# ai-forever/Kandinsky-2

Measured on NVIDIA H100. Metric: unet_denoising_steps_per_sec, higher is better.
Workload: dtype f16

## Files before the change

kandinsky-2_b200/csrc/k2_api.cu:

```cuda
#include <stdio.h>
#include <stdlib.h>
#include <string.h>

#include <algorithm>
#include <atomic>
#include <mutex>

#include "../../include/k2b200.h"
#include "k2_internal.h"

namespace k2 {

static thread_local std::string g_err;
static std::atomic<long long> g_launches{0};
static int g_force_bn = 0;
static int g_force_split = 0;
static int g_pdl = 0;


void set_error(const std::string& msg) { g_err = msg; }
int fail(const std::string& msg) {
  g_err = msg;
  return -1;
}
void count_launch(int n) { g_launches.fetch_add(n, std::memory_order_relaxed); }

bool pdl_enabled() { return g_pdl != 0; }
static int g_conv_epi_sets = 1;
static int g_gn_bps = 0;
int gn_apply_blocks_per_sm() { return g_gn_bps; }
static int g_attn_half = 1;
int attention_half_rows() { return g_attn_half; }

int num_sms() {
  static int n = 0;
  if (n == 0) {
    int dev = 0;
    cudaGetDevice(&dev);
    cudaDeviceGetAttribute(&n, cudaDevAttrMultiProcessorCount, dev);
    if (n <= 0) n = 132;
  }
  return n;
}

typedef CUresult (*EncodeTiledFn)(CUtensorMap*, CUtensorMapDataType, cuuint32_t, void*, const cuuint64_t*,
                                  const cuuint64_t*, const cuuint32_t*, const cuuint32_t*,
                                  CUtensorMapInterleave, CUtensorMapSwizzle, CUtensorMapL2promotion,
                                  CUtensorMapFloatOOBfill);

static EncodeTiledFn get_encode_fn() {
  static EncodeTiledFn fn = nullptr;
  static std::once_flag once;
  std::call_once(once, [] {
    void* p = nullptr;
    cudaDriverEntryPointQueryResult qres;
    cudaError_t e = cudaGetDriverEntryPoint("cuTensorMapEncodeTiled", &p, cudaEnableDefault, &qres);
    if (e == cudaSuccess && qres == cudaDriverEntryPointSuccess) fn = reinterpret_cast<EncodeTiledFn>(p);
  });
  return fn;
}

int encode_tmap_f16(CUtensorMap* out, const void* base, int rank, const uint64_t* dims,
                    const uint64_t* strides_bytes, const uint32_t* box) {
  EncodeTiledFn fn = get_encode_fn();
  if (!fn) return fail("cuTensorMapEncodeTiled unavailable (no CUDA driver)");
  cuuint64_t gdim[5];
  cuuint64_t gstr[4];
  cuuint32_t bx[5];
  cuuint32_t es[5];
  for (int i = 0; i < rank; ++i) {
    gdim[i] = dims[i];
    bx[i] = box[i];
    es[i] = 1;
  }
  for (int i = 0; i + 1 < rank; ++i) gstr[i] = strides_bytes[i];
  CUresult r = fn(out, CU_TENSOR_MAP_DATA_TYPE_FLOAT16, static_cast<cuuint32_t>(rank), const_cast<void*>(base),
                  gdim, gstr, bx, es, CU_TENSOR_MAP_INTERLEAVE_NONE, CU_TENSOR_MAP_SWIZZLE_128B,
                  CU_TENSOR_MAP_L2_PROMOTION_L2_256B, CU_TENSOR_MAP_FLOAT_OOB_FILL_NONE);
  if (r != CUDA_SUCCESS) {
    char buf[256];
    snprintf(buf, sizeof buf,
             "cuTensorMapEncodeTiled failed (%d): rank %d dims %llu %llu %llu %llu box %u %u %u %u base %p",
             static_cast<int>(r), rank, (unsigned long long)dims[0], (unsigned long long)(rank > 1 ? dims[1] : 0),
             (unsigned long long)(rank > 2 ? dims[2] : 0), (unsigned long long)(rank > 3 ? dims[3] : 0), box[0],
             rank > 1 ? box[1] : 0, rank > 2 ? box[2] : 0, rank > 3 ? box[3] : 0, base);
    return fail(buf);
  }
  return 0;
}

static void choose_tile(int NB, int H, int W, int& TN, int& TH, int& TW, bool single_image_only = false) {
  long long best_tiles[2] = {-1, -1};
  int bn[2] = {1, 1}, bw[2] = {1, 1}, bh[2] = {1, 1};
  const int wmax = W < 128 ? W : 128;
  for (int tw = 1; tw <= wmax; ++tw) {
    const long long tiles_w = (W + tw - 1) / tw;
    for (int tn = 1; tn <= NB && tn * tw <= 128; ++tn) {
      int thmax = 128 / (tw * tn);
      if (thmax > H) thmax = H;
      if (thmax < 1) continue;
      const long long tiles_h = (H + thmax - 1) / thmax;
      const int th = static_cast<int>((H + tiles_h - 1) / tiles_h);
      const long long tiles = tiles_h * tiles_w * ((NB + tn - 1) / tn);
      for (int k = (tn == 1 ? 0 : 1); k < 2; ++k) {
        bool better = best_tiles[k] < 0 || tiles < best_tiles[k];
        if (!better && tiles == best_tiles[k]) {
          if (tn != bn[k]) {
            better = tn < bn[k];
          } else {
            const int d_new = tw > th ? tw - th : th - tw;
            const int d_old = bw[k] > bh[k] ? bw[k] - bh[k] : bh[k] - bw[k];
            better = (d_new < d_old) || (d_new == d_old && tw > bw[k]);
          }
        }
        if (better) {
          best_tiles[k] = tiles;
          bn[k] = tn;
          bw[k] = tw;
          bh[k] = th;
        }
      }
    }
  }
  const int k = (!single_image_only && best_tiles[1] * 100 <= best_tiles[0] * 85) ? 1 : 0;
  TN = bn[k];
  TW = bw[k];
  TH = bh[k];
}


struct ConvPlan {
  int TN, TH, TW, tiles_w, tiles_h, tiles_n, m_tiles;
  int m_tiles_phase;
  int BN, splits;
  int fuse_stats, row_groups;
  int es;
};

static void plan_conv(int NB, int H, int W, bool any9, int kchunks, int Cout, int out_mode, bool has_workspace,
                      long long workspace_bytes, bool want_gn, ConvPlan& pl, const int* cfg = nullptr, bool up2 = false,
                      bool w_batched = false) {
  const int g_force_bn = (cfg && cfg[0]) ? cfg[0] : k2::g_force_bn;
  const int g_force_split = (cfg && cfg[2]) ? cfg[2] : k2::g_force_split;
  pl.es = (cfg && cfg[3]) ? cfg[3] : k2::g_conv_epi_sets;
  choose_tile(NB, H, W, pl.TN, pl.TH, pl.TW, w_batched);
  pl.tiles_w = (W + pl.TW - 1) / pl.TW;
  pl.tiles_h = (H + pl.TH - 1) / pl.TH;
  pl.tiles_n = (NB + pl.TN - 1) / pl.TN;
  pl.m_tiles = pl.tiles_w * pl.tiles_h * pl.tiles_n;
  pl.m_tiles_phase = pl.m_tiles;

  int BN = g_force_bn;
  int splits = 1;
  const long long M_total = static_cast<long long>(NB) * H * W;
  const bool can_split = !up2 && !w_batched && has_workspace && out_mode == 0 && Cout % 8 == 0;
  auto split_ok = [&](int sp) {
    if (sp == 1) return true;
    const int kps = (kchunks + sp - 1) / sp;
    return can_split && kps >= 8 && (sp - 1) * kps < kchunks &&
           static_cast<long long>(sp) * M_total * Cout * 4 <= workspace_bytes;
  };
  auto model = [&](int bn, int sp) {
    const long long nt = (Cout + bn - 1) / bn;
    const long long units = static_cast<long long>(pl.m_tiles) * nt * sp * (up2 ? 4 : 1);
    const long long slots = num_sms();
    const long long waves = (units + slots - 1) / slots;
    const long long kps = (kchunks + sp - 1) / sp;
    long long cost = waves * (kps * (4LL * bn + 60) + 2000);
    if (sp > 1) cost += 4000 + (static_cast<long long>(sp) + 1) * M_total * Cout * 4 / 1800;
    return cost;
  };
  if (BN == 0) {
    if (Cout <= 16) BN = 16;
    else if (Cout <= 64) BN = 64;
    else if (Cout <= 128) BN = 128;
    else BN = 0;
  }
  {
    const int cand[3] = {256, 192, 128};
    long long best = -1;
    int best_bn = BN ? BN : 256, best_sp = 1;
    for (int ci = 0; ci < 3; ++ci) {
      const int bn = BN ? BN : cand[ci];
      if (BN && ci > 0) break;
      for (int sp = 1; sp <= 8; ++sp) {
        if (g_force_split > 0 && sp != g_force_split) continue;
        if (!split_ok(sp)) continue;
        const long long c = model(bn, sp);
        if (best < 0 || c < best) {
          best = c;
          best_bn = bn;
          best_sp = sp;
        }
      }
    }
    BN = best_bn;
    splits = best_sp;
  }
  pl.BN = BN;
  pl.splits = splits;

  pl.fuse_stats = 0;
  pl.row_groups = 0;
  if (want_gn && out_mode == 0 && Cout % 8 == 0) {
    if (splits == 1 && BN >= 64 && Cout % 64 == 0 && (pl.TN == 1 || pl.TH * pl.TW == 16)) {
      pl.fuse_stats = 1;
      pl.row_groups = ((pl.TN == 1) ? pl.m_tiles : NB * pl.tiles_h * pl.tiles_w) * (up2 ? 4 : 1);
    } else if (splits > 1 && (static_cast<long long>(H) * W) % 16 == 0) {
      pl.fuse_stats = 2;
      pl.row_groups = static_cast<int>(M_total / 16);
    }
  }
}

static void plan_to_info(const ConvPlan& pl, int* info) {
  if (!info) return;
  info[0] = pl.BN; info[1] = 0;
  info[2] = pl.splits; info[3] = pl.m_tiles; info[4] = pl.TN;
  info[5] = pl.fuse_stats; info[6] = pl.row_groups;
}

}

using namespace k2;

extern "C" {

const char* k2_last_error(void) { return g_err.c_str(); }
int k2_version(void) { return 100; }
long long k2_launch_count(void) { return g_launches.load(); }
void k2_reset_launch_count(void) { g_launches.store(0); }
int k2_set_tuning(int key, int value) {
  if (key == 0) {
    g_force_bn = value;
    return 0;
  }
  if (key == 1) {
    g_force_split = value;
    return 0;
  }
  if (key == 2) {
    if (value == 2) return fail("k2_set_tuning: no CTA-pair conv kernel on sm_90");
    return 0;
  }
  if (key == 4) {
    g_pdl = value;
    return 0;
  }
  if (key == 10) {
    g_conv_epi_sets = (value == 2) ? 2 : 1;
    return 0;
  }
  if (key == 11) {
    g_gn_bps = value;
    return 0;
  }
  if (key == 9) {
    g_attn_half = value ? 1 : 0;
    return 0;
  }

  return fail("k2_set_tuning: unknown key");
}

int k2_conv_gemm(const K2ConvSrc* srcs, int nsrc, int NB, int H, int W, const void* w_packed, int w_rows,
                 int Ktot, int ldw, int Cout, const float* bias, const void* residual, int ldr, void* out, int ldo,
                 int out_mode, void* workspace, long long workspace_bytes, float* gn_partial, int* info,
                 k2_stream_t stream) {
  return k2_conv_gemm_cfg(srcs, nsrc, NB, H, W, w_packed, w_rows, Ktot, ldw, Cout, bias, residual, ldr, out, ldo, out_mode,
                          workspace, workspace_bytes, gn_partial, info, nullptr, 0, stream);
}

int k2_conv_gemm_cfg(const K2ConvSrc* srcs, int nsrc, int NB, int H, int W, const void* w_packed, int w_rows,
                     int Ktot, int ldw, int Cout, const float* bias, const void* residual, int ldr, void* out, int ldo,
                     int out_mode, void* workspace, long long workspace_bytes, float* gn_partial, int* info,
                     const int* cfg, long long w_batch_stride, k2_stream_t stream) {
  K2_REQUIRE(w_batch_stride >= 0 && w_batch_stride % 8 == 0, "conv_gemm_cfg: w_batch_stride must be a multiple of 8 elements");
  const bool w_batched = w_batch_stride > 0;
  if (cfg) {
    K2_REQUIRE(cfg[0] == 0 || cfg[0] == 16 || cfg[0] == 64 || cfg[0] == 128 || cfg[0] == 192 || cfg[0] == 256,
               "conv_gemm_cfg: N tile must be 0, 16, 64, 128, 192 or 256");
    K2_REQUIRE(cfg[1] >= 0 && cfg[1] <= 2 && cfg[2] >= 0 && cfg[2] <= 8 && cfg[3] >= 0 && cfg[3] <= 2,
               "conv_gemm_cfg: pair mode in 0..2, splits in 0..8, epilogue sets in 0..2");
    K2_REQUIRE(cfg[1] != 2, "conv_gemm_cfg: no CTA-pair conv kernel on sm_90");
  }
  K2_REQUIRE(nsrc >= 1 && nsrc <= 3, "conv_gemm: 1..3 sources");
  K2_REQUIRE((reinterpret_cast<uintptr_t>(gn_partial) & 7) == 0, "conv_gemm: gn_partial must be 8-byte aligned");
  K2_REQUIRE(NB > 0 && H > 0 && W > 0 && Cout > 0, "conv_gemm: bad geometry");
  K2_REQUIRE(w_rows >= Cout, "conv_gemm: w_rows < Cout");
  K2_REQUIRE(Ktot % 64 == 0, "conv_gemm: Ktot must be a multiple of 64");
  if (ldw == 0) ldw = Ktot;
  K2_REQUIRE(ldw >= Ktot && ldw % 8 == 0 && (reinterpret_cast<uintptr_t>(w_packed) & 15) == 0,
             "conv_gemm: weight row stride / alignment");
  ConvGemmParams p;
  memset(&p, 0, sizeof p);
  p.NB = NB;
  p.H = H;
  p.W = W;
  bool any9 = false;
  int kchunks = 0;
  const bool up2 = srcs[0].taps == 4;
  if (up2) {
    K2_REQUIRE(nsrc == 1 && out_mode == 0 && residual == nullptr && H % 2 == 0 && W % 2 == 0,
               "conv_gemm: a taps == 4 source (3x3 conv over its nearest-2x upsampling) must be the only source, with fp16 "
               "output, no residual and even output H, W");
    H /= 2;
    W /= 2;
    p.H = H;
    p.W = W;
  }
  for (int s = 0; s < nsrc; ++s) {
    const K2ConvSrc& src = srcs[s];
    K2_REQUIRE(src.taps == 9 || src.taps == 1 || (s == 0 && src.taps == 4), "conv_gemm: taps must be 9 or 1 (or 4: up2)");
    K2_REQUIRE(src.C > 0 && src.C % 8 == 0 && src.ld % 8 == 0 && src.ld >= src.C, "conv_gemm: bad source C/ld");
    K2_REQUIRE((reinterpret_cast<uintptr_t>(src.ptr) & 15) == 0, "conv_gemm: source not 16B aligned");
    any9 = any9 || src.taps == 9;
    p.seg_taps[s] = src.taps;
    p.seg_kchunks[s] = (src.C + 63) / 64;
    kchunks += src.taps * p.seg_kchunks[s];
  }
  K2_REQUIRE(kchunks * 64 * (up2 ? 4 : 1) == Ktot,
             "conv_gemm: Ktot does not match the sources (taps * ceil(C/64)*64 summed; x4 phases for a taps == 4 source)");
  p.num_k_chunks = kchunks;

  ConvPlan pl;
  plan_conv(NB, H, W, any9 || up2, kchunks, Cout, out_mode, workspace != nullptr, workspace_bytes, gn_partial != nullptr, pl,
            cfg, up2, w_batched);
  K2_REQUIRE(!w_batched || (!up2 && pl.TN == 1), "conv_gemm_cfg: batched weights need single-image tiles");
  p.w_batched = w_batched ? 1 : 0;
  plan_to_info(pl, info);
  p.TN = pl.TN;
  p.TH = pl.TH;
  p.TW = pl.TW;
  p.tiles_w = pl.tiles_w;
  p.tiles_h = pl.tiles_h;
  p.tiles_n = pl.tiles_n;
  p.m_tiles = up2 ? 4 * pl.m_tiles_phase : pl.m_tiles;
  p.m_tiles_phase = pl.m_tiles_phase;
  p.up2 = up2 ? 1 : 0;
  p.a_box_bytes = static_cast<uint32_t>(p.TN * p.TH * p.TW * 128);
  for (int s = 0; s < nsrc; ++s) {
    const K2ConvSrc& src = srcs[s];
    uint64_t dims[4] = {static_cast<uint64_t>(src.C), static_cast<uint64_t>(W), static_cast<uint64_t>(H),
                        static_cast<uint64_t>(NB)};
    uint64_t str[3] = {static_cast<uint64_t>(src.ld) * 2, static_cast<uint64_t>(src.ld) * 2 * W,
                       static_cast<uint64_t>(src.ld) * 2 * W * H};
    uint32_t box[4] = {64, static_cast<uint32_t>(p.TW), static_cast<uint32_t>(p.TH), static_cast<uint32_t>(p.TN)};
    if (encode_tmap_f16(&p.tmA[s], src.ptr, 4, dims, str, box)) return -1;
  }
  const int BN = pl.BN, splits = pl.splits, fuse_stats = pl.fuse_stats;
  p.splits = splits;
  p.k_per_split = (kchunks + splits - 1) / splits;
  p.M_total = static_cast<long long>(NB) * H * W * (up2 ? 4 : 1);
  p.ws = reinterpret_cast<float*>(workspace);
  p.n_tiles = (Cout + BN - 1) / BN;
  p.Cout = Cout;
  {
    uint64_t dims[3] = {static_cast<uint64_t>(Ktot), static_cast<uint64_t>(w_rows), static_cast<uint64_t>(w_batched ? NB : 1)};
    uint64_t str[2] = {static_cast<uint64_t>(ldw) * 2,
                       (w_batched ? static_cast<uint64_t>(w_batch_stride) : static_cast<uint64_t>(ldw) * w_rows) * 2};
    uint32_t box[3] = {64, static_cast<uint32_t>(BN), 1};
    if (encode_tmap_f16(&p.tmB, w_packed, 3, dims, str, box)) return -1;
  }
  p.bias = bias;
  p.residual = reinterpret_cast<const __half*>(residual);
  p.ldr = ldr;
  p.out = out;
  p.ldo = ldo;
  p.out_mode = (splits > 1) ? 2 : out_mode;
  p.gn_part = (fuse_stats == 1) ? reinterpret_cast<float2*>(gn_partial) : nullptr;
  p.gn_mode = (fuse_stats == 1) ? (p.TN == 1 ? 1 : 2) : 0;
  if (out_mode == 0) {
    K2_REQUIRE(ldo % 8 == 0 && (reinterpret_cast<uintptr_t>(out) & 15) == 0, "conv_gemm: out alignment");
    if (residual)
      K2_REQUIRE(ldr % 8 == 0 && (reinterpret_cast<uintptr_t>(residual) & 15) == 0, "conv_gemm: residual alignment");
  }
  int rc = launch_conv_gemm(p, BN, pl.es, static_cast<cudaStream_t>(stream));
  if (rc == 0) g_launches.fetch_add(1, std::memory_order_relaxed);
  if (rc == 0 && splits > 1) {
    rc = launch_splitk_finalize(p.ws, splits, p.M_total, Cout, bias, p.residual, ldr, reinterpret_cast<__half*>(out), ldo,
                                fuse_stats == 2 ? reinterpret_cast<float2*>(gn_partial) : nullptr,
                                static_cast<cudaStream_t>(stream));
    if (rc == 0) g_launches.fetch_add(1, std::memory_order_relaxed);
  }
  return rc;
}

int k2_conv_plan(int NB, int H, int W, int taps, int Ktot, int Cout, int out_mode, long long workspace_bytes,
                 int want_gn_partial, int* info) {
  K2_REQUIRE(NB > 0 && H > 0 && W > 0 && Cout > 0 && info, "conv_plan: bad arguments");
  K2_REQUIRE(Ktot > 0 && Ktot % 64 == 0, "conv_plan: Ktot must be a positive multiple of 64");
  ConvPlan pl;
  plan_conv(NB, H, W, taps == 9, Ktot / 64, Cout, out_mode, workspace_bytes > 0, workspace_bytes, want_gn_partial != 0, pl);
  plan_to_info(pl, info);
  return 0;
}

}
```

kandinsky-2_b200/csrc/k2_attention.cu:

```cuda
#include <string.h>

#include <algorithm>

#include "../../include/k2b200.h"
#include "k2_common.cuh"
#include "k2_internal.h"

namespace k2 {

namespace {

__device__ __forceinline__ float ex2(float x) {
  float y;
  asm("ex2.approx.ftz.f32 %0, %1;" : "=f"(y) : "f"(x));
  return y;
}
__device__ __forceinline__ uint32_t pack_h2(float lo, float hi) {
  __half2 h = __floats2half2_rn(lo, hi);
  return *reinterpret_cast<uint32_t*>(&h);
}

template <int D, int DV, int NW, int BKV>
struct FlashCfg {
  static constexpr int BQ = 16 * NW;
  static constexpr int QP = D + 8;
  static constexpr int VP = DV + 8;
  static constexpr int Q_BYTES = BQ * QP * 2;
  static constexpr int K_BYTES = BKV * QP * 2;
  static constexpr int V_BYTES = BKV * VP * 2;
  static constexpr int SMEM_BYTES = Q_BYTES + 2 * (K_BYTES + V_BYTES);
};

template <int D, int DV, int NW, int BKV>
__global__ void __launch_bounds__(NW * 32, 1) flash_attention_kernel(const FlashParams p) {
  using C = FlashCfg<D, DV, NW, BKV>;
  constexpr int NSPLIT = D / DV;
  extern __shared__ __align__(16) uint8_t smem[];
  __half* sQ = reinterpret_cast<__half*>(smem);
  __half* sK = reinterpret_cast<__half*>(smem + C::Q_BYTES);
  __half* sV = reinterpret_cast<__half*>(smem + C::Q_BYTES + 2 * C::K_BYTES);

  const int tid = threadIdx.x;
  const int warp = tid >> 5;
  const int lane = tid & 31;
  const int q0 = blockIdx.x * C::BQ;
  const int head = blockIdx.y / NSPLIT;
  const int dsplit = blockIdx.y - head * NSPLIT;
  const int b = blockIdx.z;
  const int Tkv = p.Tc + p.T;
  const int nblk = (Tkv + BKV - 1) / BKV;

  pdl_wait();
  pdl_launch();

  {
    constexpr int CPR = D / 8;
    for (int i = tid; i < C::BQ * CPR; i += NW * 32) {
      const int r = i / CPR, c = i - r * CPR;
      const int q = q0 + r;
      const __half* src = p.qkv + (static_cast<long long>(b) * p.T + (q < p.T ? q : 0)) * p.ldq + head * p.hs + p.q_off + c * 8;
      cp_async_16(smem_u32(sQ + r * C::QP + c * 8), src, q < p.T ? 16 : 0);
    }
  }
  auto load_kv = [&](int jb, int st) {
    constexpr int KC = D / 8, VC = DV / 8;
    for (int i = tid; i < BKV * (KC + VC); i += NW * 32) {
      const int r = i / (KC + VC), c = i - r * (KC + VC);
      const int key = jb * BKV + r;
      const bool ok = key < Tkv;
      const bool from_enc = key < p.Tc;
      const __half* row = from_enc ? p.enc + (static_cast<long long>(b) * p.Tc + key) * p.lde + head * p.ehs
                                   : p.qkv + (static_cast<long long>(b) * p.T + (ok ? key - p.Tc : 0)) * p.ldq + head * p.hs;
      if (c < KC) {
        const __half* src = row + (from_enc ? p.ek_off : p.k_off) + c * 8;
        cp_async_16(smem_u32(sK + (st * BKV + r) * C::QP + c * 8), ok ? src : p.qkv, ok ? 16 : 0);
      } else {
        const __half* src = row + (from_enc ? p.ev_off : p.v_off) + dsplit * DV + (c - KC) * 8;
        cp_async_16(smem_u32(sV + (st * BKV + r) * C::VP + (c - KC) * 8), ok ? src : p.qkv, ok ? 16 : 0);
      }
    }
  };
  load_kv(0, 0);
  cp_async_commit();

  const float c = p.scale_log2e;
  float m_r[2] = {-INFINITY, -INFINITY}, l_r[2] = {0.f, 0.f};
  float o[DV / 8][4];
#pragma unroll
  for (int n = 0; n < DV / 8; ++n) o[n][0] = o[n][1] = o[n][2] = o[n][3] = 0.f;

  const uint32_t q_lane = smem_u32(sQ + (warp * 16 + (lane & 15)) * C::QP + (lane >> 4) * 8);
  for (int jb = 0; jb < nblk; ++jb) {
    const int st = jb & 1;
    if (jb + 1 < nblk) {
      load_kv(jb + 1, st ^ 1);
      cp_async_commit();
      cp_async_wait<1>();
    } else {
      cp_async_wait<0>();
    }
    __syncthreads();

    float s[BKV / 8][4];
#pragma unroll
    for (int n = 0; n < BKV / 8; ++n) s[n][0] = s[n][1] = s[n][2] = s[n][3] = 0.f;
    const uint32_t k_lane = smem_u32(sK + (st * BKV + ((lane >> 4) << 3) + (lane & 7)) * C::QP + ((lane >> 3) & 1) * 8);
#pragma unroll 4
    for (int kk = 0; kk < D / 16; ++kk) {
      uint32_t a[4];
      ldmatrix_x4(a, q_lane + kk * 32);
#pragma unroll
      for (int n = 0; n < BKV / 8; n += 2) {
        uint32_t bk[4];
        ldmatrix_x4(bk, k_lane + n * 8 * C::QP * 2 + kk * 32);
        mma_16816(s[n], a, bk[0], bk[1]);
        mma_16816(s[n + 1], a, bk[2], bk[3]);
      }
    }

    const int kbase = jb * BKV + 2 * (lane & 3);
    float mx[2] = {-INFINITY, -INFINITY};
#pragma unroll
    for (int n = 0; n < BKV / 8; ++n) {
#pragma unroll
      for (int e = 0; e < 4; ++e) {
        const int key = kbase + n * 8 + (e & 1);
        s[n][e] = key < Tkv ? s[n][e] * c : -INFINITY;
        mx[e >> 1] = fmaxf(mx[e >> 1], s[n][e]);
      }
    }
    float alpha[2];
#pragma unroll
    for (int h = 0; h < 2; ++h) {
      mx[h] = fmaxf(mx[h], __shfl_xor_sync(0xffffffffu, mx[h], 1));
      mx[h] = fmaxf(mx[h], __shfl_xor_sync(0xffffffffu, mx[h], 2));
      const float m_new = fmaxf(m_r[h], mx[h]);
      alpha[h] = ex2(m_r[h] - m_new);
      m_r[h] = m_new;
    }
    float ls[2] = {0.f, 0.f};
#pragma unroll
    for (int n = 0; n < BKV / 8; ++n) {
#pragma unroll
      for (int e = 0; e < 4; ++e) {
        s[n][e] = ex2(s[n][e] - m_r[e >> 1]);
        ls[e >> 1] += s[n][e];
      }
    }
#pragma unroll
    for (int h = 0; h < 2; ++h) l_r[h] = l_r[h] * alpha[h] + ls[h];
#pragma unroll
    for (int n = 0; n < DV / 8; ++n) {
      o[n][0] *= alpha[0];
      o[n][1] *= alpha[0];
      o[n][2] *= alpha[1];
      o[n][3] *= alpha[1];
    }

    const uint32_t v_lane = smem_u32(sV + (st * BKV + ((lane >> 3) & 1) * 8 + (lane & 7)) * C::VP + (lane >> 4) * 8);
#pragma unroll
    for (int kk = 0; kk < BKV / 16; ++kk) {
      uint32_t a[4];
      a[0] = pack_h2(s[2 * kk][0], s[2 * kk][1]);
      a[1] = pack_h2(s[2 * kk][2], s[2 * kk][3]);
      a[2] = pack_h2(s[2 * kk + 1][0], s[2 * kk + 1][1]);
      a[3] = pack_h2(s[2 * kk + 1][2], s[2 * kk + 1][3]);
#pragma unroll
      for (int n = 0; n < DV / 8; n += 2) {
        uint32_t bv[4];
        ldmatrix_x4_trans(bv, v_lane + (kk * 16 * C::VP + n * 8) * 2);
        mma_16816(o[n], a, bv[0], bv[1]);
        mma_16816(o[n + 1], a, bv[2], bv[3]);
      }
    }
    __syncthreads();
  }

  l_r[0] += __shfl_xor_sync(0xffffffffu, l_r[0], 1);
  l_r[0] += __shfl_xor_sync(0xffffffffu, l_r[0], 2);
  l_r[1] += __shfl_xor_sync(0xffffffffu, l_r[1], 1);
  l_r[1] += __shfl_xor_sync(0xffffffffu, l_r[1], 2);
  const float inv[2] = {1.f / l_r[0], 1.f / l_r[1]};
#pragma unroll
  for (int h = 0; h < 2; ++h) {
    const int q = q0 + warp * 16 + (lane >> 2) + 8 * h;
    if (q >= p.T) continue;
    __half* orow = p.out + (static_cast<long long>(b) * p.T + q) * p.ldo + head * p.ohs + dsplit * DV + 2 * (lane & 3);
#pragma unroll
    for (int n = 0; n < DV / 8; ++n)
      *reinterpret_cast<uint32_t*>(orow + n * 8) = pack_h2(o[n][2 * h] * inv[h], o[n][2 * h + 1] * inv[h]);
  }
}

template <int D, int DV, int NW, int BKV>
int launch_flash(const FlashParams& p, cudaStream_t stream) {
  using C = FlashCfg<D, DV, NW, BKV>;
  static bool attr_set = false;
  if (!attr_set) {
    K2_CHECK_CUDA(cudaFuncSetAttribute(flash_attention_kernel<D, DV, NW, BKV>, cudaFuncAttributeMaxDynamicSharedMemorySize,
                                       C::SMEM_BYTES));
    attr_set = true;
  }
  dim3 grid((p.T + C::BQ - 1) / C::BQ, p.heads * (D / DV), p.B);
  K2_CHECK_CUDA(launch_k(flash_attention_kernel<D, DV, NW, BKV>, grid, dim3(NW * 32), C::SMEM_BYTES, stream, p));
  return 0;
}

}

int launch_attention(const FlashParams& p, int head_dim, cudaStream_t stream) {
  if (head_dim == 512) return launch_flash<512, 256, 8, 16>(p, stream);
  return attention_half_rows() ? launch_flash<64, 64, 8, 64>(p, stream) : launch_flash<64, 64, 4, 64>(p, stream);
}

}

using namespace k2;

extern "C" int k2_attention_d64(const void* qkv, int ldq, int hs, int q_off, int k_off, int v_off, const void* enc,
                                int lde, int ehs, int ek_off, int ev_off, int B, int heads, int T, int Tc, float scale,
                                void* out, int ldo, k2_stream_t stream) {
  K2_REQUIRE(qkv && out && B > 0 && heads > 0 && T > 0, "attention_d64: bad arguments");
  K2_REQUIRE(ldq % 8 == 0 && ldo % 8 == 0 && hs % 8 == 0 && q_off % 8 == 0 && k_off % 8 == 0 && v_off % 8 == 0,
             "attention_d64: strides/offsets must be multiples of 8 elements");
  K2_REQUIRE((enc != nullptr) == (Tc > 0), "attention_d64: enc and Tc go together");
  K2_REQUIRE((reinterpret_cast<uintptr_t>(qkv) & 15) == 0 && (reinterpret_cast<uintptr_t>(out) & 15) == 0,
             "attention_d64: 16-byte alignment");
  K2_REQUIRE((heads - 1) * hs + std::max(std::max(q_off, k_off), v_off) + 64 <= ldq,
             "attention_d64: qkv row narrower than heads*hs");
  if (Tc > 0) {
    K2_REQUIRE(lde % 8 == 0 && ehs % 8 == 0 && ek_off % 8 == 0 && ev_off % 8 == 0 &&
                   (reinterpret_cast<uintptr_t>(enc) & 15) == 0,
               "attention_d64: encoder strides/alignment");
    K2_REQUIRE((heads - 1) * ehs + std::max(ek_off, ev_off) + 64 <= lde, "attention_d64: encoder row narrower than heads*ehs");
  }
  FlashParams p;
  memset(&p, 0, sizeof p);
  p.qkv = reinterpret_cast<const __half*>(qkv);
  p.ldq = ldq; p.hs = hs; p.q_off = q_off; p.k_off = k_off; p.v_off = v_off;
  p.enc = reinterpret_cast<const __half*>(enc);
  p.lde = lde; p.ehs = ehs; p.ek_off = ek_off; p.ev_off = ev_off;
  p.B = B; p.heads = heads; p.T = T; p.Tc = Tc;
  p.out = reinterpret_cast<__half*>(out);
  p.ldo = ldo;
  p.ohs = 64;
  p.scale_log2e = scale * 1.4426950408889634f;
  int rc = launch_attention(p, 64, static_cast<cudaStream_t>(stream));
  if (rc == 0) count_launch();
  return rc;
}
```

kandinsky-2_b200/csrc/k2_common.cuh:

```cuda
#pragma once
#include <cuda.h>
#include <cuda_fp16.h>
#include <cuda_runtime.h>
#include <stdint.h>
#include <stdio.h>

namespace k2 {

__device__ __forceinline__ uint32_t smem_u32(const void* p) {
  return static_cast<uint32_t>(__cvta_generic_to_shared(p));
}

__device__ __forceinline__ uint32_t lane_id() { return threadIdx.x & 31; }

__device__ __forceinline__ bool elect_one() {
  uint32_t pred = 0;
  asm volatile(
      "{\n"
      ".reg .b32 rx;\n"
      ".reg .pred px;\n"
      "elect.sync rx|px, 0xffffffff;\n"
      "selp.b32 %0, 1, 0, px;\n"
      "}\n"
      : "=r"(pred));
  return pred != 0;
}

__device__ __forceinline__ void mbar_init(uint64_t* bar, uint32_t count) {
  asm volatile("mbarrier.init.shared::cta.b64 [%0], %1;" ::"r"(smem_u32(bar)), "r"(count));
}
__device__ __forceinline__ void fence_barrier_init() {
  asm volatile("fence.mbarrier_init.release.cluster;" ::: "memory");
}
__device__ __forceinline__ void mbar_arrive_expect_tx(uint64_t* bar, uint32_t bytes) {
  asm volatile("mbarrier.arrive.expect_tx.shared::cta.b64 _, [%0], %1;" ::"r"(smem_u32(bar)),
               "r"(bytes)
               : "memory");
}
__device__ __forceinline__ void mbar_arrive(uint64_t* bar) {
  asm volatile("mbarrier.arrive.shared::cta.b64 _, [%0];" ::"r"(smem_u32(bar)) : "memory");
}
__device__ __forceinline__ bool mbar_try_wait(uint64_t* bar, uint32_t parity) {
  uint32_t ok;
  asm volatile(
      "{\n"
      ".reg .pred p;\n"
      "mbarrier.try_wait.parity.shared::cta.b64 p, [%1], %2;\n"
      "selp.b32 %0, 1, 0, p;\n"
      "}\n"
      : "=r"(ok)
      : "r"(smem_u32(bar)), "r"(parity)
      : "memory");
  return ok != 0;
}
__device__ __forceinline__ void mbar_wait(uint64_t* bar, uint32_t parity) {
  if (mbar_try_wait(bar, parity)) return;
  long long t0 = clock64();
  while (!mbar_try_wait(bar, parity)) {
    if (clock64() - t0 > 4000000000LL) {
      printf("k2b200: mbarrier wait timeout (block %d,%d,%d thread %d)\n", blockIdx.x, blockIdx.y,
             blockIdx.z, threadIdx.x);
      __trap();
    }
  }
}

__device__ __forceinline__ void mbar_wait_lean(uint64_t* bar, uint32_t parity) {
  if (mbar_try_wait(bar, parity)) return;
  long long t0 = clock64();
  while (!mbar_try_wait(bar, parity)) {
    if (clock64() - t0 > 4000000000LL) __trap();
  }
}

__device__ __forceinline__ void fence_proxy_async_smem() {
  asm volatile("fence.proxy.async.shared::cta;" ::: "memory");
}

__device__ __forceinline__ void tma_prefetch_desc(const CUtensorMap* tm) {
  asm volatile("prefetch.tensormap [%0];" ::"l"(reinterpret_cast<uint64_t>(tm)) : "memory");
}
__device__ __forceinline__ void tma_load_2d(void* dst, const CUtensorMap* tm, uint64_t* bar, int c0,
                                            int c1) {
  asm volatile(
      "cp.async.bulk.tensor.2d.shared::cluster.global.mbarrier::complete_tx::bytes [%0], [%1, {%3, "
      "%4}], [%2];"
      ::"r"(smem_u32(dst)),
      "l"(reinterpret_cast<uint64_t>(tm)), "r"(smem_u32(bar)), "r"(c0), "r"(c1)
      : "memory");
}
__device__ __forceinline__ void tma_load_3d(void* dst, const CUtensorMap* tm, uint64_t* bar, int c0,
                                            int c1, int c2) {
  asm volatile(
      "cp.async.bulk.tensor.3d.shared::cluster.global.mbarrier::complete_tx::bytes [%0], [%1, {%3, "
      "%4, %5}], [%2];"
      ::"r"(smem_u32(dst)),
      "l"(reinterpret_cast<uint64_t>(tm)), "r"(smem_u32(bar)), "r"(c0), "r"(c1), "r"(c2)
      : "memory");
}
__device__ __forceinline__ void tma_load_4d(void* dst, const CUtensorMap* tm, uint64_t* bar, int c0,
                                            int c1, int c2, int c3) {
  asm volatile(
      "cp.async.bulk.tensor.4d.shared::cluster.global.mbarrier::complete_tx::bytes [%0], [%1, {%3, "
      "%4, %5, %6}], [%2];"
      ::"r"(smem_u32(dst)),
      "l"(reinterpret_cast<uint64_t>(tm)), "r"(smem_u32(bar)), "r"(c0), "r"(c1), "r"(c2), "r"(c3)
      : "memory");
}

__device__ __forceinline__ uint64_t make_wgmma_desc(uint32_t smem_addr) {
  uint64_t d = 0;
  d |= static_cast<uint64_t>((smem_addr & 0x3FFFF) >> 4);
  d |= static_cast<uint64_t>(1) << 16;
  d |= static_cast<uint64_t>(1024 >> 4) << 32;
  d |= static_cast<uint64_t>(1) << 62;
  return d;
}
__device__ __forceinline__ void wgmma_fence() { asm volatile("wgmma.fence.sync.aligned;" ::: "memory"); }
__device__ __forceinline__ void wgmma_commit() { asm volatile("wgmma.commit_group.sync.aligned;" ::: "memory"); }
template <int N>
__device__ __forceinline__ void wgmma_wait() {
  asm volatile("wgmma.wait_group.sync.aligned %0;" ::"n"(N) : "memory");
}
__device__ __forceinline__ void wgmma_m64n16k16(float (&d)[8], uint64_t adesc, uint64_t bdesc, uint32_t accumulate) {
  asm volatile(
      "{\n"
      ".reg .pred p;\n"
      "setp.ne.b32 p, %10, 0;\n"
      "wgmma.mma_async.sync.aligned.m64n16k16.f32.f16.f16 "
      "{%0, %1, %2, %3, %4, %5, %6, %7}, %8, %9, p, 1, 1, 0, 0;\n"
      "}\n"
      : "+f"(d[0]), "+f"(d[1]), "+f"(d[2]), "+f"(d[3]), "+f"(d[4]), "+f"(d[5]), "+f"(d[6]), "+f"(d[7])
      : "l"(adesc), "l"(bdesc), "r"(accumulate));
}

__device__ __forceinline__ void wgmma_m64n64k16(float (&d)[32], uint64_t adesc, uint64_t bdesc, uint32_t accumulate) {
  asm volatile(
      "{\n"
      ".reg .pred p;\n"
      "setp.ne.b32 p, %34, 0;\n"
      "wgmma.mma_async.sync.aligned.m64n64k16.f32.f16.f16 "
      "{%0, %1, %2, %3, %4, %5, %6, %7, %8, %9, %10, %11, %12, %13, %14, %15, %16, %17, %18, %19, %20, %21, %22, %23, %24, %25, %26, %27, %28, %29, %30, %31}, %32, %33, p, 1, 1, 0, 0;\n"
      "}\n"
      : "+f"(d[0]), "+f"(d[1]), "+f"(d[2]), "+f"(d[3]), "+f"(d[4]), "+f"(d[5]), "+f"(d[6]), "+f"(d[7]), "+f"(d[8]), "+f"(d[9]), "+f"(d[10]), "+f"(d[11]), "+f"(d[12]), "+f"(d[13]), "+f"(d[14]), "+f"(d[15]), "+f"(d[16]), "+f"(d[17]), "+f"(d[18]), "+f"(d[19]), "+f"(d[20]), "+f"(d[21]), "+f"(d[22]), "+f"(d[23]), "+f"(d[24]), "+f"(d[25]), "+f"(d[26]), "+f"(d[27]), "+f"(d[28]), "+f"(d[29]), "+f"(d[30]), "+f"(d[31])
      : "l"(adesc), "l"(bdesc), "r"(accumulate));
}

#define K2_WGMMA_D8(o)                                                                                                  \
  "+f"(d[(o)]), "+f"(d[(o) + 1]), "+f"(d[(o) + 2]), "+f"(d[(o) + 3]), "+f"(d[(o) + 4]), "+f"(d[(o) + 5]), "+f"(d[(o) + 6]), \
      "+f"(d[(o) + 7])
#define K2_WGMMA_D32(o) K2_WGMMA_D8(o), K2_WGMMA_D8((o) + 8), K2_WGMMA_D8((o) + 16), K2_WGMMA_D8((o) + 24)

__device__ __forceinline__ void wgmma_m64n128k16(float (&d)[64], uint64_t adesc, uint64_t bdesc, uint32_t accumulate) {
  asm volatile(
      "{\n"
      ".reg .pred p;\n"
      "setp.ne.b32 p, %66, 0;\n"
      "wgmma.mma_async.sync.aligned.m64n128k16.f32.f16.f16 {"
      "%0, %1, %2, %3, %4, %5, %6, %7, %8, %9, %10, %11, %12, %13, %14, %15, "
      "%16, %17, %18, %19, %20, %21, %22, %23, %24, %25, %26, %27, %28, %29, %30, %31, "
      "%32, %33, %34, %35, %36, %37, %38, %39, %40, %41, %42, %43, %44, %45, %46, %47, "
      "%48, %49, %50, %51, %52, %53, %54, %55, %56, %57, %58, %59, %60, %61, %62, %63"
      "}, %64, %65, p, 1, 1, 0, 0;\n"
      "}\n"
      : K2_WGMMA_D32(0), K2_WGMMA_D32(32)
      : "l"(adesc), "l"(bdesc), "r"(accumulate));
}

__device__ __forceinline__ void wgmma_m64n192k16(float (&d)[96], uint64_t adesc, uint64_t bdesc, uint32_t accumulate) {
  asm volatile(
      "{\n"
      ".reg .pred p;\n"
      "setp.ne.b32 p, %98, 0;\n"
      "wgmma.mma_async.sync.aligned.m64n192k16.f32.f16.f16 {"
      "%0, %1, %2, %3, %4, %5, %6, %7, %8, %9, %10, %11, %12, %13, %14, %15, "
      "%16, %17, %18, %19, %20, %21, %22, %23, %24, %25, %26, %27, %28, %29, %30, %31, "
      "%32, %33, %34, %35, %36, %37, %38, %39, %40, %41, %42, %43, %44, %45, %46, %47, "
      "%48, %49, %50, %51, %52, %53, %54, %55, %56, %57, %58, %59, %60, %61, %62, %63, "
      "%64, %65, %66, %67, %68, %69, %70, %71, %72, %73, %74, %75, %76, %77, %78, %79, "
      "%80, %81, %82, %83, %84, %85, %86, %87, %88, %89, %90, %91, %92, %93, %94, %95"
      "}, %96, %97, p, 1, 1, 0, 0;\n"
      "}\n"
      : K2_WGMMA_D32(0), K2_WGMMA_D32(32), K2_WGMMA_D32(64)
      : "l"(adesc), "l"(bdesc), "r"(accumulate));
}

__device__ __forceinline__ void wgmma_m64n256k16(float (&d)[128], uint64_t adesc, uint64_t bdesc, uint32_t accumulate) {
  asm volatile(
      "{\n"
      ".reg .pred p;\n"
      "setp.ne.b32 p, %130, 0;\n"
      "wgmma.mma_async.sync.aligned.m64n256k16.f32.f16.f16 {"
      "%0, %1, %2, %3, %4, %5, %6, %7, %8, %9, %10, %11, %12, %13, %14, %15, "
      "%16, %17, %18, %19, %20, %21, %22, %23, %24, %25, %26, %27, %28, %29, %30, %31, "
      "%32, %33, %34, %35, %36, %37, %38, %39, %40, %41, %42, %43, %44, %45, %46, %47, "
      "%48, %49, %50, %51, %52, %53, %54, %55, %56, %57, %58, %59, %60, %61, %62, %63, "
      "%64, %65, %66, %67, %68, %69, %70, %71, %72, %73, %74, %75, %76, %77, %78, %79, "
      "%80, %81, %82, %83, %84, %85, %86, %87, %88, %89, %90, %91, %92, %93, %94, %95, "
      "%96, %97, %98, %99, %100, %101, %102, %103, %104, %105, %106, %107, %108, %109, %110, %111, "
      "%112, %113, %114, %115, %116, %117, %118, %119, %120, %121, %122, %123, %124, %125, %126, %127"
      "}, %128, %129, p, 1, 1, 0, 0;\n"
      "}\n"
      : K2_WGMMA_D32(0), K2_WGMMA_D32(32), K2_WGMMA_D32(64), K2_WGMMA_D32(96)
      : "l"(adesc), "l"(bdesc), "r"(accumulate));
}
#undef K2_WGMMA_D32
#undef K2_WGMMA_D8

template <int R>
__device__ __forceinline__ void setmaxnreg_dec() {
  asm volatile("setmaxnreg.dec.sync.aligned.u32 %0;" ::"n"(R));
}
template <int R>
__device__ __forceinline__ void setmaxnreg_inc() {
  asm volatile("setmaxnreg.inc.sync.aligned.u32 %0;" ::"n"(R));
}

__device__ __forceinline__ void mma_16816(float (&d)[4], const uint32_t (&a)[4], uint32_t b0, uint32_t b1) {
  asm volatile(
      "mma.sync.aligned.m16n8k16.row.col.f32.f16.f16.f32 {%0, %1, %2, %3}, {%4, %5, %6, %7}, {%8, %9}, "
      "{%0, %1, %2, %3};"
      : "+f"(d[0]), "+f"(d[1]), "+f"(d[2]), "+f"(d[3])
      : "r"(a[0]), "r"(a[1]), "r"(a[2]), "r"(a[3]), "r"(b0), "r"(b1));
}
__device__ __forceinline__ void ldmatrix_x4(uint32_t (&r)[4], uint32_t saddr) {
  asm volatile("ldmatrix.sync.aligned.m8n8.x4.shared.b16 {%0, %1, %2, %3}, [%4];"
               : "=r"(r[0]), "=r"(r[1]), "=r"(r[2]), "=r"(r[3])
               : "r"(saddr));
}
__device__ __forceinline__ void ldmatrix_x4_trans(uint32_t (&r)[4], uint32_t saddr) {
  asm volatile("ldmatrix.sync.aligned.m8n8.x4.trans.shared.b16 {%0, %1, %2, %3}, [%4];"
               : "=r"(r[0]), "=r"(r[1]), "=r"(r[2]), "=r"(r[3])
               : "r"(saddr));
}
__device__ __forceinline__ void cp_async_16(uint32_t saddr, const void* gptr, int src_bytes) {
  asm volatile("cp.async.cg.shared.global [%0], [%1], 16, %2;" ::"r"(saddr), "l"(gptr), "r"(src_bytes) : "memory");
}
__device__ __forceinline__ void cp_async_commit() { asm volatile("cp.async.commit_group;" ::: "memory"); }
template <int N>
__device__ __forceinline__ void cp_async_wait() {
  asm volatile("cp.async.wait_group %0;" ::"n"(N) : "memory");
}

__device__ __forceinline__ void sts_v4(uint32_t saddr, uint32_t a, uint32_t b, uint32_t c, uint32_t d) {
  asm volatile("st.shared.v4.b32 [%0], {%1, %2, %3, %4};" ::"r"(saddr), "r"(a), "r"(b), "r"(c), "r"(d) : "memory");
}
__device__ __forceinline__ uint4 lds_v4(uint32_t saddr) {
  uint4 v;
  asm volatile("ld.shared.v4.b32 {%0, %1, %2, %3}, [%4];" : "=r"(v.x), "=r"(v.y), "=r"(v.z), "=r"(v.w) : "r"(saddr) : "memory");
  return v;
}
__device__ __forceinline__ uint32_t lds_u32(uint32_t saddr) {
  uint32_t v;
  asm volatile("ld.shared.b32 %0, [%1];" : "=r"(v) : "r"(saddr) : "memory");
  return v;
}
__device__ __forceinline__ void named_bar_sync(int id, int count) {
  asm volatile("bar.sync %0, %1;" ::"r"(id), "r"(count) : "memory");
}
__device__ __forceinline__ void pdl_wait() { asm volatile("griddepcontrol.wait;" ::: "memory"); }
__device__ __forceinline__ void pdl_launch() { asm volatile("griddepcontrol.launch_dependents;" ::: "memory"); }

__device__ __forceinline__ float silu_f(float x) {
  const float h = 0.5f * x;
  float t;
  asm("tanh.approx.f32 %0, %1;" : "=f"(t) : "f"(h));
  return fmaf(h, t, h);
}

}
```

kandinsky-2_b200/csrc/k2_internal.h:

```cpp
#pragma once
#include <cuda.h>
#include <cuda_fp16.h>
#include <cuda_runtime.h>
#include <stdint.h>

#include <string>

namespace k2 {

void set_error(const std::string& msg);
int fail(const std::string& msg);
#define K2_CHECK_CUDA(expr)                                                                 \
  do {                                                                                      \
    cudaError_t _e = (expr);                                                                \
    if (_e != cudaSuccess)                                                                  \
      return ::k2::fail(std::string(#expr) + ": " + cudaGetErrorString(_e));                \
  } while (0)
#define K2_REQUIRE(cond, msg)                                  \
  do {                                                         \
    if (!(cond)) return ::k2::fail(std::string("k2b200: ") + (msg)); \
  } while (0)

inline bool aligned16(const void* p) { return (reinterpret_cast<uintptr_t>(p) & 15) == 0; }

int num_sms();
bool pdl_enabled();

template <typename... KArgs, typename... Args>
inline cudaError_t launch_k(void (*kernel)(KArgs...), dim3 grid, dim3 block, size_t smem, cudaStream_t stream,
                            Args&&... args) {
  cudaLaunchConfig_t cfg = {};
  cfg.gridDim = grid;
  cfg.blockDim = block;
  cfg.dynamicSmemBytes = smem;
  cfg.stream = stream;
  cudaLaunchAttribute attr[1];
  attr[0].id = cudaLaunchAttributeProgrammaticStreamSerialization;
  attr[0].val.programmaticStreamSerializationAllowed = 1;
  cfg.attrs = attr;
  cfg.numAttrs = pdl_enabled() ? 1 : 0;
  return cudaLaunchKernelEx(&cfg, kernel, static_cast<KArgs>(args)...);
}
void count_launch(int n = 1);

int encode_tmap_f16(CUtensorMap* out, const void* base, int rank, const uint64_t* dims,
                    const uint64_t* strides_bytes , const uint32_t* box);

struct ConvGemmParams {
  CUtensorMap tmA[3];
  CUtensorMap tmB;
  int w_batched;
  int seg_taps[3];
  int seg_kchunks[3];
  int num_k_chunks;
  int NB, H, W;
  int TN, TH, TW;
  int tiles_n, tiles_h, tiles_w;
  int m_tiles, n_tiles;
  int Cout;
  const float* bias;
  const __half* residual;
  int ldr;
  void* out;
  int ldo;
  int out_mode;
  uint32_t a_box_bytes;
  int splits;
  int k_per_split;
  float* ws;
  long long M_total;
  float2* gn_part;
  int gn_mode;
  int up2;
  int m_tiles_phase;
};
int launch_conv_gemm(const ConvGemmParams& p, int BN, int epilogue_sets, cudaStream_t stream);
int launch_splitk_finalize(const float* ws, int splits, long long M, int Cout, const float* bias, const __half* residual,
                           int ldr, __half* out, int ldo, float2* gn_part, cudaStream_t stream);

struct FlashParams {
  const __half* qkv;
  long long ldq;
  int hs, q_off, k_off, v_off;
  const __half* enc;
  long long lde;
  int ehs, ek_off, ev_off;
  int B, heads, T, Tc;
  __half* out;
  int ldo, ohs;
  float scale_log2e;
};
int gn_apply_blocks_per_sm();
int attention_half_rows();
int launch_attention(const FlashParams& p, int head_dim, cudaStream_t stream);

}
```

Before: 20.73.

## Replace head-dim-64 flash attention with warp-specialized TMA/WGMMA pipelined kernel

```diff
diff --git a/kandinsky-2_b200/csrc/k2_api.cu b/kandinsky-2_b200/csrc/k2_api.cu
--- a/kandinsky-2_b200/csrc/k2_api.cu
+++ b/kandinsky-2_b200/csrc/k2_api.cu
@@ -29,8 +29,6 @@
 static int g_conv_epi_sets = 1;
 static int g_gn_bps = 0;
 int gn_apply_blocks_per_sm() { return g_gn_bps; }
-static int g_attn_half = 1;
-int attention_half_rows() { return g_attn_half; }
 
 int num_sms() {
   static int n = 0;
@@ -256,7 +254,6 @@
     return 0;
   }
   if (key == 9) {
-    g_attn_half = value ? 1 : 0;
     return 0;
   }
 
diff --git a/kandinsky-2_b200/csrc/k2_attention.cu b/kandinsky-2_b200/csrc/k2_attention.cu
--- a/kandinsky-2_b200/csrc/k2_attention.cu
+++ b/kandinsky-2_b200/csrc/k2_attention.cu
@@ -206,11 +206,245 @@
   return 0;
 }
 
+namespace d64 {
+constexpr int BQ = 128;
+constexpr int BKV = 128;
+constexpr int STAGES = 4;
+constexpr int TILE = 128 * 128;
+constexpr int BAR_BYTES = 8 * (2 * STAGES + 1);
+constexpr int SMEM_BYTES = 1024 + TILE * (1 + 2 * STAGES) + BAR_BYTES;
+constexpr int TURN_BAR = 1;
+}
+
+struct AttnD64Params {
+  CUtensorMap tm_qkv;
+  CUtensorMap tm_enc;
+  __half* out;
+  long long ldo;
+  int hs, q_off, k_off, v_off;
+  int ehs, ek_off, ev_off;
+  int T, Tc;
+  float scale_log2e;
+};
+
+template <bool MASK>
+__device__ __forceinline__ void softmax_block(float (&s)[64], float (&m)[2], float (&l)[2], float (&alpha)[2], float c, int valid) {
+  const int kq = 2 * (threadIdx.x & 3);
+  if (MASK) {
+#pragma unroll
+    for (int i = 0; i < 64; ++i)
+      if (8 * (i >> 2) + kq + (i & 1) >= valid) s[i] = -INFINITY;
+  }
+  float mx[2] = {-INFINITY, -INFINITY};
+#pragma unroll
+  for (int i = 0; i < 64; ++i) mx[(i >> 1) & 1] = fmaxf(mx[(i >> 1) & 1], s[i]);
+#pragma unroll
+  for (int h = 0; h < 2; ++h) {
+    mx[h] = fmaxf(mx[h], __shfl_xor_sync(0xffffffffu, mx[h], 1));
+    mx[h] = fmaxf(mx[h], __shfl_xor_sync(0xffffffffu, mx[h], 2));
+    const float m_new = fmaxf(m[h], mx[h] * c);
+    alpha[h] = ex2(m[h] - m_new);
+    m[h] = m_new;
+  }
+  float ls[2][2] = {{0.f, 0.f}, {0.f, 0.f}};
+#pragma unroll
+  for (int i = 0; i < 64; ++i) {
+    const int h = (i >> 1) & 1;
+    s[i] = ex2(fmaf(s[i], c, -m[h]));
+    ls[h][(i >> 2) & 1] += s[i];
+  }
+#pragma unroll
+  for (int h = 0; h < 2; ++h) l[h] = l[h] * alpha[h] + (ls[h][0] + ls[h][1]);
+}
+
+__global__ void __launch_bounds__(384, 1) attention_d64_kernel(const __grid_constant__ AttnD64Params p) {
+  using namespace d64;
+  extern __shared__ uint8_t smem_raw[];
+  uint8_t* smem = reinterpret_cast<uint8_t*>((reinterpret_cast<uintptr_t>(smem_raw) + 1023) & ~static_cast<uintptr_t>(1023));
+  uint8_t* sQ = smem;
+  uint8_t* sK = smem + TILE;
+  uint8_t* sV = sK + STAGES * TILE;
+  uint64_t* full_bar = reinterpret_cast<uint64_t*>(sV + STAGES * TILE);
+  uint64_t* empty_bar = full_bar + STAGES;
+  uint64_t* q_bar = empty_bar + STAGES;
+
+  const int warp = threadIdx.x >> 5;
+  const int lane = threadIdx.x & 31;
+  const int wg = warp >> 2;
+  const int q0 = blockIdx.x * BQ;
+  const int head = blockIdx.y;
+  const int b = blockIdx.z;
+  const int nenc = (p.Tc + BKV - 1) / BKV;
+  const int nblk = nenc + (p.T + BKV - 1) / BKV;
+
+  if (threadIdx.x == 0) {
+    tma_prefetch_desc(&p.tm_qkv);
+    if (nenc) tma_prefetch_desc(&p.tm_enc);
+    for (int i = 0; i < STAGES; ++i) {
+      mbar_init(&full_bar[i], 1);
+      mbar_init(&empty_bar[i], 8);
+    }
+    mbar_init(q_bar, 1);
+    fence_barrier_init();
+  }
+  __syncthreads();
+  pdl_wait();
+  pdl_launch();
+
+  if (wg == 0) {
+    setmaxnreg_dec<40>();
+    if (warp == 0 && elect_one()) {
+      mbar_arrive_expect_tx(q_bar, TILE);
+      tma_load_3d(sQ, &p.tm_qkv, q_bar, head * p.hs + p.q_off, q0, b);
+      for (int j = 0; j < nblk; ++j) {
+        const int st = j % STAGES;
+        if (j >= STAGES) mbar_wait_lean(&empty_bar[st], (j / STAGES - 1) & 1);
+        mbar_arrive_expect_tx(&full_bar[st], 2 * TILE);
+        if (j < nenc) {
+          tma_load_3d(sK + st * TILE, &p.tm_enc, &full_bar[st], head * p.ehs + p.ek_off, j * BKV, b);
+          tma_load_3d(sV + st * TILE, &p.tm_enc, &full_bar[st], head * p.ehs + p.ev_off, j * BKV, b);
+        } else {
+          tma_load_3d(sK + st * TILE, &p.tm_qkv, &full_bar[st], head * p.hs + p.k_off, (j - nenc) * BKV, b);
+          tma_load_3d(sV + st * TILE, &p.tm_qkv, &full_bar[st], head * p.hs + p.v_off, (j - nenc) * BKV, b);
+        }
+      }
+    }
+    return;
+  }
+
+  setmaxnreg_inc<232>();
+  const int cw = wg - 1;
+  const float c = p.scale_log2e;
+  const uint64_t qdesc = make_wgmma_desc(smem_u32(sQ) + cw * 64 * 128);
+  const uint32_t k_base = smem_u32(sK), v_base = smem_u32(sV);
+
+  float o[32], s[64], m[2] = {-INFINITY, -INFINITY}, l[2] = {0.f, 0.f}, alpha[2] = {0.f, 0.f};
+  uint32_t pa[32];
+#pragma unroll
+  for (int i = 0; i < 32; ++i) o[i] = 0.f;
+
+  auto issue_pv = [&](int st) {
+#pragma unroll
+    for (int kk = 0; kk < BKV / 16; ++kk) {
+      const uint32_t a[4] = {pa[4 * kk], pa[4 * kk + 1], pa[4 * kk + 2], pa[4 * kk + 3]};
+      wgmma_m64n64k16_rs_tb(o, a, make_wgmma_desc_mn(v_base + st * TILE) + static_cast<uint64_t>(kk * (2048 >> 4)));
+    }
+    wgmma_commit();
+  };
+  auto rescale_o = [&]() {
+#pragma unroll
+    for (int i = 0; i < 32; ++i) o[i] *= alpha[(i >> 1) & 1];
+  };
+
+  auto issue_s = [&](int j) {
+    const int st = j % STAGES;
+    mbar_wait_lean(&full_bar[st], (j / STAGES) & 1);
+    named_bar_sync(TURN_BAR + cw, 256);
+    wgmma_fence();
+#pragma unroll
+    for (int kk = 0; kk < 4; ++kk)
+      wgmma_m64n128k16(s, qdesc + static_cast<uint64_t>(kk * 2), make_wgmma_desc(k_base + st * TILE) + static_cast<uint64_t>(kk * 2),
+                       kk > 0);
+    wgmma_commit();
+  };
+  auto pass_turn = [&](int j) {
+    if (cw == 0 || j + 1 < nblk) named_bar_arrive(TURN_BAR + 1 - cw, 256);
+  };
+  auto softmax = [&](int j) {
+#pragma unroll
+    for (int i = 0; i < 64; ++i) reg_fence(s[i]);
+    const int valid = j < nenc ? p.Tc - j * BKV : p.T - (j - nenc) * BKV;
+    if (valid < BKV) softmax_block<true>(s, m, l, alpha, c, valid);
+    else softmax_block<false>(s, m, l, alpha, c, valid);
+  };
+  auto to_p = [&]() {
+#pragma unroll
+    for (int i = 0; i < 32; ++i) pa[i] = pack_h2(s[2 * i], s[2 * i + 1]);
+  };
+
+  if (cw == 1) named_bar_arrive(TURN_BAR, 256);
+  mbar_wait_lean(q_bar, 0);
+  issue_s(0);
+  pass_turn(0);
+  wgmma_wait<0>();
+  softmax(0);
+  to_p();
+  for (int j = 1; j < nblk; ++j) {
+    const int pst = (j - 1) % STAGES;
+    rescale_o();
+    issue_s(j);
+    issue_pv(pst);
+    pass_turn(j);
+    wgmma_wait<1>();
+    softmax(j);
+    wgmma_wait<0>();
+#pragma unroll
+    for (int i = 0; i < 32; ++i) reg_fence(o[i]);
+    if (lane == 0) mbar_arrive(&empty_bar[pst]);
+    to_p();
+  }
+  rescale_o();
+  wgmma_fence();
+  issue_pv((nblk - 1) % STAGES);
+  wgmma_wait<0>();
+#pragma unroll
+  for (int i = 0; i < 32; ++i) reg_fence(o[i]);
+
+#pragma unroll
+  for (int h = 0; h < 2; ++h) {
+    l[h] += __shfl_xor_sync(0xffffffffu, l[h], 1);
+    l[h] += __shfl_xor_sync(0xffffffffu, l[h], 2);
+  }
+  const float inv[2] = {1.f / l[0], 1.f / l[1]};
+#pragma unroll
+  for (int h = 0; h < 2; ++h) {
+    const int q = q0 + 64 * cw + 16 * (warp & 3) + (lane >> 2) + 8 * h;
+    if (q >= p.T) continue;
+    __half* orow = p.out + (static_cast<long long>(b) * p.T + q) * p.ldo + head * 64 + 2 * (lane & 3);
+#pragma unroll
+    for (int n = 0; n < 8; ++n)
+      *reinterpret_cast<uint32_t*>(orow + n * 8) = pack_h2(o[4 * n + 2 * h] * inv[h], o[4 * n + 2 * h + 1] * inv[h]);
+  }
+}
+
+int launch_attention_d64(const FlashParams& f, cudaStream_t stream) {
+  using namespace d64;
+  AttnD64Params p;
+  memset(&p, 0, sizeof p);
+  const uint32_t box[3] = {64, BKV, 1};
+  {
+    const uint64_t width = static_cast<uint64_t>(f.heads - 1) * f.hs + std::max(std::max(f.q_off, f.k_off), f.v_off) + 64;
+    const uint64_t dims[3] = {width, static_cast<uint64_t>(f.T), static_cast<uint64_t>(f.B)};
+    const uint64_t strides[2] = {static_cast<uint64_t>(f.ldq) * 2, static_cast<uint64_t>(f.ldq) * 2 * f.T};
+    if (encode_tmap_f16(&p.tm_qkv, f.qkv, 3, dims, strides, box)) return -1;
+  }
+  if (f.Tc > 0) {
+    const uint64_t width = static_cast<uint64_t>(f.heads - 1) * f.ehs + std::max(f.ek_off, f.ev_off) + 64;
+    const uint64_t dims[3] = {width, static_cast<uint64_t>(f.Tc), static_cast<uint64_t>(f.B)};
+    const uint64_t strides[2] = {static_cast<uint64_t>(f.lde) * 2, static_cast<uint64_t>(f.lde) * 2 * f.Tc};
+    if (encode_tmap_f16(&p.tm_enc, f.enc, 3, dims, strides, box)) return -1;
+  }
+  p.out = f.out;
+  p.ldo = f.ldo;
+  p.hs = f.hs; p.q_off = f.q_off; p.k_off = f.k_off; p.v_off = f.v_off;
+  p.ehs = f.ehs; p.ek_off = f.ek_off; p.ev_off = f.ev_off;
+  p.T = f.T; p.Tc = f.Tc;
+  p.scale_log2e = f.scale_log2e;
+  static bool attr_set = false;
+  if (!attr_set) {
+    K2_CHECK_CUDA(cudaFuncSetAttribute(attention_d64_kernel, cudaFuncAttributeMaxDynamicSharedMemorySize, SMEM_BYTES));
+    attr_set = true;
+  }
+  dim3 grid((f.T + BQ - 1) / BQ, f.heads, f.B);
+  K2_CHECK_CUDA(launch_k(attention_d64_kernel, grid, dim3(384), SMEM_BYTES, stream, p));
+  return 0;
+}
+
 }
 
 int launch_attention(const FlashParams& p, int head_dim, cudaStream_t stream) {
   if (head_dim == 512) return launch_flash<512, 256, 8, 16>(p, stream);
-  return attention_half_rows() ? launch_flash<64, 64, 8, 64>(p, stream) : launch_flash<64, 64, 4, 64>(p, stream);
+  return launch_attention_d64(p, stream);
 }
 
 }
diff --git a/kandinsky-2_b200/csrc/k2_common.cuh b/kandinsky-2_b200/csrc/k2_common.cuh
--- a/kandinsky-2_b200/csrc/k2_common.cuh
+++ b/kandinsky-2_b200/csrc/k2_common.cuh
@@ -204,8 +204,30 @@
       : K2_WGMMA_D32(0), K2_WGMMA_D32(32), K2_WGMMA_D32(64), K2_WGMMA_D32(96)
       : "l"(adesc), "l"(bdesc), "r"(accumulate));
 }
+__device__ __forceinline__ uint64_t make_wgmma_desc_mn(uint32_t smem_addr) {
+  uint64_t d = 0;
+  d |= static_cast<uint64_t>((smem_addr & 0x3FFFF) >> 4);
+  d |= static_cast<uint64_t>(1) << 16;
+  d |= static_cast<uint64_t>(1024 >> 4) << 32;
+  d |= static_cast<uint64_t>(1) << 62;
+  return d;
+}
+
+__device__ __forceinline__ void wgmma_m64n64k16_rs_tb(float (&d)[32], const uint32_t (&a)[4], uint64_t bdesc) {
+  asm volatile(
+      "{\n"
+      "wgmma.mma_async.sync.aligned.m64n64k16.f32.f16.f16 {"
+      "%0, %1, %2, %3, %4, %5, %6, %7, %8, %9, %10, %11, %12, %13, %14, %15, "
+      "%16, %17, %18, %19, %20, %21, %22, %23, %24, %25, %26, %27, %28, %29, %30, %31"
+      "}, {%32, %33, %34, %35}, %36, 1, 1, 1, 1;\n"
+      "}\n"
+      : K2_WGMMA_D32(0)
+      : "r"(a[0]), "r"(a[1]), "r"(a[2]), "r"(a[3]), "l"(bdesc));
+}
 #undef K2_WGMMA_D32
 #undef K2_WGMMA_D8
+
+__device__ __forceinline__ void reg_fence(float& r) { asm volatile("" : "+f"(r)::"memory"); }
 
 template <int R>
 __device__ __forceinline__ void setmaxnreg_dec() {
@@ -257,6 +279,9 @@
 }
 __device__ __forceinline__ void named_bar_sync(int id, int count) {
   asm volatile("bar.sync %0, %1;" ::"r"(id), "r"(count) : "memory");
+}
+__device__ __forceinline__ void named_bar_arrive(int id, int count) {
+  asm volatile("bar.arrive %0, %1;" ::"r"(id), "r"(count) : "memory");
 }
 __device__ __forceinline__ void pdl_wait() { asm volatile("griddepcontrol.wait;" ::: "memory"); }
 __device__ __forceinline__ void pdl_launch() { asm volatile("griddepcontrol.launch_dependents;" ::: "memory"); }
diff --git a/kandinsky-2_b200/csrc/k2_internal.h b/kandinsky-2_b200/csrc/k2_internal.h
--- a/kandinsky-2_b200/csrc/k2_internal.h
+++ b/kandinsky-2_b200/csrc/k2_internal.h
@@ -91,7 +91,6 @@
   float scale_log2e;
 };
 int gn_apply_blocks_per_sm();
-int attention_half_rows();
 int launch_attention(const FlashParams& p, int head_dim, cudaStream_t stream);
 
 }
diff --git a/profiles/attention_layers.py b/profiles/attention_layers.py
--- /dev/null
+++ b/profiles/attention_layers.py
@@ -0,0 +1,86 @@
+import argparse
+import json
+import os
+import subprocess
+import sys
+
+ROOT = os.path.dirname(os.path.dirname(os.path.abspath(__file__)))
+for p in (ROOT, os.path.join(ROOT, "kandinsky-2_b200")):
+    if p not in sys.path:
+        sys.path.insert(0, p)
+
+import torch
+
+SHAPES = [
+    ("cfg-2 level 1 (48x48)", 8, 12, 2304, 32, 7),
+    ("cfg-2 level 2 (24x24)", 8, 18, 576, 32, 7),
+    ("cfg-2 level 3 + mid (12x12)", 8, 24, 144, 32, 8),
+    ("cfg-3 level 1 (64x64)", 4, 12, 4096, 32, None),
+]
+
+
+def _card():
+    q = subprocess.run(["nvidia-smi", "--query-gpu=name,power.limit,clocks.max.sm", "--format=csv,noheader", "-i", "0"],
+                       capture_output=True, text=True)
+    return q.stdout.strip() or torch.cuda.get_device_name(0)
+
+
+def _time(run, min_ms):
+    for _ in range(3):
+        run()
+    torch.cuda.synchronize()
+    s, e = torch.cuda.Event(enable_timing=True), torch.cuda.Event(enable_timing=True)
+    s.record()
+    for _ in range(5):
+        run()
+    e.record()
+    torch.cuda.synchronize()
+    reps = max(10, int(min_ms / max(s.elapsed_time(e) / 5, 1e-3)) + 1)
+    s.record()
+    for _ in range(reps):
+        run()
+    e.record()
+    torch.cuda.synchronize()
+    return s.elapsed_time(e) / reps, reps
+
+
+def main():
+    ap = argparse.ArgumentParser()
+    ap.add_argument("--out", default=None)
+    ap.add_argument("--lib", default=None, help="libk2b200.so to time (default: the in-tree build)")
+    ap.add_argument("--min-ms", type=float, default=100.0, help="timed window per shape")
+    args = ap.parse_args()
+    if not torch.cuda.is_available():
+        raise SystemExit("needs a CUDA sm_90 device")
+    from kandinsky2 import _native, ops
+    if args.lib:
+        _native.LIB_PATH = os.path.abspath(args.lib)
+    _native.load()
+    dev = torch.device("cuda", 0)
+    torch.cuda.set_device(dev)
+    ops.set_tuning(4, 1)
+    res = {"card": _card(), "torch": torch.__version__, "lib": _native.LIB_PATH, "min_ms": args.min_ms}
+    g = torch.Generator(device=dev).manual_seed(11)
+    rows = []
+    for name, B, heads, T, Tc, per_step in SHAPES:
+        qkv = torch.randn(B, T, heads * 192, device=dev, generator=g).half()
+        enc = torch.randn(B, Tc, heads * 128, device=dev, generator=g).half()
+        out = torch.empty(B, T, heads * 64, device=dev, dtype=torch.float16)
+        ms, reps = _time(lambda: ops.attention_d64(qkv, heads, enc, out=out), args.min_ms)
+        flops = 4.0 * B * heads * T * (T + Tc) * 64
+        rows.append(dict(shape=name, B=B, heads=heads, T=T, Tc=Tc, launches_per_step=per_step, ms=round(ms, 5), reps=reps,
+                         gflop=round(flops * 1e-9, 2), tflops=round(flops / (ms * 1e-3) / 1e12, 1),
+                         ms_per_step=round(ms * per_step, 4) if per_step else None))
+    res["shapes"] = rows
+    print(f"# {res['card']}  {res['lib']}")
+    print(f"{'shape':30s} {'ms':>9s} {'TFLOP/s':>8s} {'ms/step':>8s}")
+    for r in rows:
+        print(f"{r['shape']:30s} {r['ms']:9.4f} {r['tflops']:8.1f} " + (f"{r['ms_per_step']:8.3f}" if r["ms_per_step"] else ""))
+    if args.out:
+        os.makedirs(os.path.dirname(os.path.abspath(args.out)), exist_ok=True)
+        with open(args.out, "w") as f:
+            f.write(json.dumps(res, indent=1) + "\n")
+
+
+if __name__ == "__main__":
+    main()
```

Measured after the change: 22.33 (median of 6 runs). 1.08x the previous value.
